# zju-pi/diff-sampler

Measured on NVIDIA H100. Metric: images/sec at fixed NFE, higher is better.
Workload: dtype fp16 operands, fp32 accumulate (split-precision: fp16 hi x hi + two e4m3 correction MMAs per product); 1 GPU; EDM cifar10 U-Net, heun num_steps=10 (NFE=18), batch 512/GPU; net=cifar10, solver=heun, nfe=18, batch_per_gpu=512, global_batch=512, weights=random init (reference constructors, seed 0), init_zero layers de-zeroed, parallelism=dp1, l2=per-forward activation working set (GBs) >> 50 MB L2

## Files before the change

### diff-sampler_b200/_lib.py

```python
import ctypes as C
import os

import torch

from . import _cstructs as S

_HERE = os.path.dirname(os.path.abspath(__file__))
LIB_PATH = os.path.join(_HERE, 'libdiffsampler_b200.so')

EXPORTS = [
    'ds_version', 'ds_last_error', 'ds_weights_create', 'ds_weights_destroy', 'ds_unet_create', 'ds_unet_destroy',
    'ds_unet_forward', 'ds_unet_debug_read', 'ds_unet_last_launch_count', 'ds_solver_update', 'ds_dyn_threshold',
    'ds_op_launch', 'ds_sizeof', 'ds_unet_set_profiling', 'ds_unet_get_profile', 'ds_unet_op_type', 'ds_gits_cost', 'ds_unet_forward_io', 'ds_images_to_uint8', 'ds_solver_update_u8', 'ds_unet_enable_graph', 'ds_amed_predict',
    'ds_gemm_config', 'ds_op_check',
]

_lib = None


class DsError(RuntimeError):
    pass


def load():
    global _lib
    if _lib is not None:
        return _lib
    if not os.path.exists(LIB_PATH):
        raise DsError(f'{LIB_PATH} not found: build it with `python diff-sampler_b200/build.py` '
                      '(there is no CPU fallback for the CUDA path)')
    lib = C.CDLL(LIB_PATH)
    vp, cp, sz = C.c_void_p, C.c_char_p, C.c_size_t
    lib.ds_version.restype = cp
    lib.ds_last_error.restype = cp
    lib.ds_weights_create.argtypes = [vp, sz, C.POINTER(vp)]
    lib.ds_weights_destroy.argtypes = [vp]
    lib.ds_weights_destroy.restype = None
    lib.ds_unet_create.argtypes = [vp, vp, C.c_int, sz, sz, C.POINTER(vp)]
    lib.ds_unet_destroy.argtypes = [vp]
    lib.ds_unet_destroy.restype = None
    lib.ds_unet_forward.argtypes = [vp, vp, vp, vp, vp, vp, vp]
    lib.ds_unet_forward_io.argtypes = [vp, C.POINTER(vp), C.c_int, vp]
    lib.ds_unet_enable_graph.argtypes = [vp, C.POINTER(sz), C.c_int]
    lib.ds_unet_debug_read.argtypes = [vp, sz, vp, sz, vp]
    lib.ds_unet_last_launch_count.argtypes = [vp]
    lib.ds_unet_set_profiling.argtypes = [vp, C.c_int]
    lib.ds_unet_get_profile.argtypes = [vp, C.POINTER(C.c_float), C.c_int]
    lib.ds_unet_op_type.argtypes = [vp, C.c_int]
    lib.ds_solver_update.argtypes = [vp, vp, vp, vp, vp, C.POINTER(vp), C.c_int, vp, C.c_int, C.c_float, vp,
                                     C.POINTER(C.c_float), vp, C.c_int64, C.c_int, vp]
    lib.ds_solver_update_u8.argtypes = [vp, vp, vp, C.c_int, C.c_int, vp, vp, vp, C.POINTER(vp), C.c_int, vp, C.c_int, C.c_float, vp,
                                        C.POINTER(C.c_float), vp, C.c_int64, C.c_int, vp]
    lib.ds_amed_predict.argtypes = [vp, C.POINTER(C.c_int), vp, vp, vp, C.c_float, C.c_float, vp, C.c_int, vp]
    lib.ds_dyn_threshold.argtypes = [vp, vp, C.c_int, C.c_int, C.c_float, C.c_float, vp]
    lib.ds_gits_cost.argtypes = [vp, vp, vp, vp, C.c_int, C.c_int, C.c_int64, vp]
    lib.ds_images_to_uint8.argtypes = [vp, vp, C.c_int, C.c_int, C.c_int, vp]
    lib.ds_op_launch.argtypes = [C.c_int, vp, sz, vp]
    lib.ds_op_check.argtypes = [C.c_int, vp, sz]
    lib.ds_sizeof.argtypes = [C.c_int]
    lib.ds_sizeof.restype = sz
    lib.ds_gemm_config.argtypes = [vp, C.POINTER(C.c_int)]
    for which, cls in S.SIZEOF_CHECKS.items():
        got, want = C.sizeof(cls), lib.ds_sizeof(which)
        if got != want:
            raise DsError(f'struct mirror {cls.__name__}: ctypes size {got} != library size {want}')
    _lib = lib
    return lib


def check(rc, what=''):
    if rc != 0:
        msg = load().ds_last_error().decode()
        raise DsError(f'{what} failed (rc={rc}): {msg}')


def version():
    return load().ds_version().decode()


def op_launch(desc, stream=0):
    lib = load()
    check(lib.ds_op_launch(S.OP_TYPE_OF[type(desc)], C.byref(desc), C.sizeof(desc), C.c_void_p(stream)), type(desc).__name__)


def op_check(desc):
    lib = load()
    if lib.ds_op_check(S.OP_TYPE_OF[type(desc)], C.byref(desc), C.sizeof(desc)) == 0:
        return None
    return lib.ds_last_error().decode()


def gemm_config(desc):
    info = (C.c_int * 2)()
    check(load().ds_gemm_config(C.byref(desc), info), 'ds_gemm_config')
    return dict(stages=info[0], grid=info[1])


class NativePlans:

    def __init__(self, blob, device):
        self.lib = load()
        self.device = device
        self.plans = {}
        self._wh = C.c_void_p()
        with torch.cuda.device(device):
            check(self.lib.ds_weights_create(blob, len(blob), C.byref(self._wh)), 'ds_weights_create')

    def get(self, key, compile_fn, io_bytes=None):
        ent = self.plans.get(key)
        if ent is None:
            pl = compile_fn()
            h = C.c_void_p()
            with torch.cuda.device(self.device):
                check(self.lib.ds_unet_create(self._wh, C.cast(pl.ops_array, C.c_void_p), pl.n_ops, C.sizeof(S.PlanOp), pl.arena_bytes,
                                              C.byref(h)), 'ds_unet_create')
                if io_bytes is not None:
                    check(self.lib.ds_unet_enable_graph(h, (C.c_size_t * S.DS_IO_COUNT)(*io_bytes(pl)), S.DS_IO_COUNT),
                          'ds_unet_enable_graph')
            ent = self.plans[key] = (h, pl)
        return ent

    def run(self, h, io, stream):
        check(self.lib.ds_unet_forward_io(h, (C.c_void_p * S.DS_IO_COUNT)(*io), S.DS_IO_COUNT, C.c_void_p(stream)), 'ds_unet_forward_io')
        return self.lib.ds_unet_last_launch_count(h)

    def debug_read(self, key, name, numel, dtype=torch.float32):
        h, pl = self.plans[key]
        t = torch.empty(numel, dtype=dtype)
        stream = torch.cuda.current_stream(self.device).cuda_stream
        check(self.lib.ds_unet_debug_read(h, pl.arena_offsets[name], t.data_ptr(), t.numel() * t.element_size(), C.c_void_p(stream)),
              'ds_unet_debug_read')
        return t

    def __del__(self):
        try:
            for h, _ in self.plans.values():
                self.lib.ds_unet_destroy(h)
            self.lib.ds_weights_destroy(self._wh)
        except Exception:
            pass
```

### diff-sampler_b200/csrc/gemm_tc.cu

```cuda
#include "ops.h"
#include "ptx.cuh"
#include <cuda_fp16.h>
#include <stdio.h>
#include <stdlib.h>
#include <string.h>

namespace dsb {

static constexpr int kMaxStages = 8;
static constexpr int kATileBytes = 128 * 128;
static constexpr int kThreads = 384;
static constexpr int kStgPitch = 64;
static constexpr int kStgBytes = 2 * 64 * kStgPitch * 4;
static constexpr int kSmemLimit = 227 * 1024;

struct alignas(64) GemmKernelParams {
    CUtensorMap tmA, tmA2, tmB;
    CUtensorMap tmA8, tmA2_8, tmB8;
    int f8, cpb8, nkb8_main, nkb8_aux, a8_plane_n;
    float acc_scale;
    int BN, m_tiles, n_tiles, num_z, nh;
    int taps, cpb, nkb_main, nkb_aux, npass;
    int a_mode, conv_H, conv_W, a_bn_dummy;
    int a_plane_n, a2_plane_n, b_plane_batch;
    int a_c_per_zh, a_n_per_zb, a_n_per_zh;
    int b_k0, b_k_per_zh, b_row_per_zh, b_z_per_zb, b_z_per_zh;
    int m_valid, n_valid;
    int num_stages;
    float* out_f32;
    __half* out_h16;
    long long o_zb, o_zh, ldo, o_plane;
    const float* bias_n;
    const float* bias_m;
    const float* rowvec;
    long long rowvec_stride;
    int rows_per_sample;
    const float* residual;
    long long ldr;
    float scale;
    int edm_out;
    const float* edm_x;
    const float* edm_coef;
    int edm_coef_stride;
    int edm_C;
    float* edm_D;
    float* st_quads;
    int st_unit;
    int tap_dh[9], tap_dw[9], tap_cb[9];
    int f8_last_steps;
};

struct SmemCtl {
    uint64_t full[kMaxStages];
    uint64_t empty[kMaxStages];
};

template <int N>
__device__ __forceinline__ void warp_sum_levels(float* v, int lane, int off) {
    if constexpr (N >= 1) {
        const bool up = (lane & off) != 0;
#pragma unroll
        for (int i = 0; i < N; ++i) {
            const float send = up ? v[i] : v[i + N];
            const float keep = up ? v[i + N] : v[i];
            v[i] = keep + __shfl_xor_sync(0xffffffffu, send, off);
        }
        warp_sum_levels<N / 2>(v, lane, off >> 1);
    } else {
        for (; off >= 1; off >>= 1) v[0] += __shfl_xor_sync(0xffffffffu, v[0], off);
    }
}
template <int NV>
__device__ __forceinline__ void warp_sum_multi(float (&v)[NV], int lane) {
    static_assert(NV == 32 || NV == 16 || NV == 8, "NV");
    warp_sum_levels<NV / 2>(v, lane, 16);
}

template <int W>
__device__ __forceinline__ void epilogue_chunk(const GemmKernelParams& p, const float* v, long long grow_in_z, int col0, bool row_ok,
                                               int zb, int zh) {
    const bool warp_rows_ok = __all_sync(0xffffffffu, row_ok);
    if (!row_ok) return;
    float r[W];
#pragma unroll
    for (int j = 0; j < W; ++j) r[j] = v[j] * p.acc_scale;
    const bool full = (col0 + W <= p.n_valid);
    if (p.bias_n) {
        if (full) {
#pragma unroll
            for (int j = 0; j < W; j += 4) {
                const float4 t = __ldg(reinterpret_cast<const float4*>(p.bias_n + col0 + j));
                r[j] += t.x; r[j + 1] += t.y; r[j + 2] += t.z; r[j + 3] += t.w;
            }
        } else {
#pragma unroll
            for (int j = 0; j < W; ++j)
                if (col0 + j < p.n_valid) r[j] += __ldg(p.bias_n + col0 + j);
        }
    }
    if (p.bias_m) {
        const float bm = __ldg(p.bias_m + grow_in_z);
#pragma unroll
        for (int j = 0; j < W; ++j) r[j] += bm;
    }
    if (p.rowvec) {
        const long long s = (p.rowvec_stride == 0) ? 0 : (grow_in_z / p.rows_per_sample) * p.rowvec_stride;
        const float* rv = p.rowvec + s + col0;
        if (full) {
#pragma unroll
            for (int j = 0; j < W; j += 4) {
                const float4 t = __ldg(reinterpret_cast<const float4*>(rv + j));
                r[j] += t.x; r[j + 1] += t.y; r[j + 2] += t.z; r[j + 3] += t.w;
            }
        } else {
#pragma unroll
            for (int j = 0; j < W; ++j)
                if (col0 + j < p.n_valid) r[j] += __ldg(rv + j);
        }
    }
    if (p.residual) {
        const float* rs = p.residual + grow_in_z * p.ldr + col0;
        if (full) {
#pragma unroll
            for (int j = 0; j < W; j += 4) {
                const float4 t = *reinterpret_cast<const float4*>(rs + j);
                r[j] += t.x; r[j + 1] += t.y; r[j + 2] += t.z; r[j + 3] += t.w;
            }
        } else {
#pragma unroll
            for (int j = 0; j < W; ++j)
                if (col0 + j < p.n_valid) r[j] += rs[j];
        }
    }
#pragma unroll
    for (int j = 0; j < W; ++j) r[j] *= p.scale;

    if (p.st_quads) {
        const int lane = threadIdx.x & 31;
        if (p.st_unit == 2) {
            float q[W];
#pragma unroll
            for (int j = 0; j < W; j += 2) {
                q[j] = r[j] + r[j + 1];
                q[j + 1] = fmaf(r[j], r[j], r[j + 1] * r[j + 1]);
            }
            warp_sum_multi<W>(q, lane);
            constexpr int kShift = (W == 32) ? 0 : 1;
            const int vi = lane >> kShift;
            if ((lane & ((1 << kShift) - 1)) == 0 && col0 + 2 * (vi >> 1) < p.n_valid)
                p.st_quads[(grow_in_z >> 5) * (long long)p.n_valid + col0 + vi] = q[0];
        } else {
            float q[W / 2];
#pragma unroll
            for (int j = 0; j < W; j += 4) {
                q[j / 2] = (r[j] + r[j + 1]) + (r[j + 2] + r[j + 3]);
                q[j / 2 + 1] = fmaf(r[j], r[j], r[j + 1] * r[j + 1]) + fmaf(r[j + 2], r[j + 2], r[j + 3] * r[j + 3]);
            }
            warp_sum_multi<W / 2>(q, lane);
            constexpr int kShift = (W == 32) ? 1 : 2;
            const int vi = lane >> kShift;
            if ((lane & ((1 << kShift) - 1)) == 0 && col0 + 4 * (vi >> 1) < p.n_valid)
                p.st_quads[((grow_in_z >> 5) * (long long)(p.n_valid >> 2)) * 2 + (col0 >> 1) + vi] = q[0];
        }
    }

    if (p.edm_out) {
        const int HW = p.rows_per_sample;
        const long long n = grow_in_z / HW;
        const long long hw = grow_in_z % HW;
        if (p.edm_out == 2) {
#pragma unroll
            for (int j = 0; j < W; ++j) {
                const int c = col0 + j;
                if (c < p.edm_C) p.edm_D[(n * p.edm_C + c) * HW + hw] = r[j];
            }
            return;
        }
        const float cskip = __ldg(p.edm_coef + n * p.edm_coef_stride + 0);
        const float cout = __ldg(p.edm_coef + n * p.edm_coef_stride + 1);
#pragma unroll
        for (int j = 0; j < W; ++j) {
            const int c = col0 + j;
            if (c < p.edm_C) {
                const long long idx = (n * p.edm_C + c) * HW + hw;
                p.edm_D[idx] = cskip * __ldg(p.edm_x + idx) + cout * r[j];
            }
        }
        return;
    }

    const long long obase = (long long)zb * p.o_zb + (long long)zh * p.o_zh + grow_in_z * p.ldo + col0;
    const int odd = threadIdx.x & 1;
    if (p.out_f32) {
        float* o = p.out_f32 + obase;
        if (full && warp_rows_ok) {
            float* oe = o - odd * p.ldo + odd * 4;
#pragma unroll
            for (int j = 0; j < W; j += 8) {
                float x[4];
#pragma unroll
                for (int k = 0; k < 4; ++k) x[k] = __shfl_xor_sync(0xffffffffu, odd ? r[j + k] : r[j + 4 + k], 1);
                const float4 s1 = odd ? make_float4(x[0], x[1], x[2], x[3]) : make_float4(r[j], r[j + 1], r[j + 2], r[j + 3]);
                const float4 s2 = odd ? make_float4(r[j + 4], r[j + 5], r[j + 6], r[j + 7]) : make_float4(x[0], x[1], x[2], x[3]);
                *reinterpret_cast<float4*>(oe + j) = s1;
                *reinterpret_cast<float4*>(oe + p.ldo + j) = s2;
            }
        } else if (full) {
#pragma unroll
            for (int j = 0; j < W; j += 4) *reinterpret_cast<float4*>(o + j) = make_float4(r[j], r[j + 1], r[j + 2], r[j + 3]);
        } else {
#pragma unroll
            for (int j = 0; j < W; ++j)
                if (col0 + j < p.n_valid) o[j] = r[j];
        }
    }
    if (p.out_h16) {
        __half* oh = p.out_h16 + obase;
        if (full) {
            __align__(16) __half hi[W];
            __align__(16) __half lo[W];
#pragma unroll
            for (int j = 0; j < W; ++j) {
                hi[j] = __float2half_rn(r[j]);
                lo[j] = __float2half_rn(r[j] - __half2float(hi[j]));
            }
            if (warp_rows_ok && W % 16 == 0) {
                __half* he = oh - odd * p.ldo + odd * 8;
#pragma unroll
                for (int pl = 0; pl < 2; ++pl) {
                    if (pl == 1 && !p.o_plane) break;
                    const __half* src = pl ? lo : hi;
                    __half* dst = he + (pl ? p.o_plane : 0);
#pragma unroll
                    for (int j = 0; j < W; j += 16) {
                        const uint4 a = *reinterpret_cast<const uint4*>(src + j), b = *reinterpret_cast<const uint4*>(src + j + 8);
                        const uint4 snd = odd ? a : b;
                        uint4 x;
                        x.x = __shfl_xor_sync(0xffffffffu, snd.x, 1); x.y = __shfl_xor_sync(0xffffffffu, snd.y, 1);
                        x.z = __shfl_xor_sync(0xffffffffu, snd.z, 1); x.w = __shfl_xor_sync(0xffffffffu, snd.w, 1);
                        *reinterpret_cast<uint4*>(dst + j) = odd ? x : a;
                        *reinterpret_cast<uint4*>(dst + p.ldo + j) = odd ? b : x;
                    }
                }
            } else {
#pragma unroll
                for (int j = 0; j < W; j += 8) *reinterpret_cast<uint4*>(oh + j) = *reinterpret_cast<const uint4*>(hi + j);
                if (p.o_plane) {
#pragma unroll
                    for (int j = 0; j < W; j += 8)
                        *reinterpret_cast<uint4*>(oh + p.o_plane + j) = *reinterpret_cast<const uint4*>(lo + j);
                }
            }
        } else {
#pragma unroll
            for (int j = 0; j < W; ++j)
                if (col0 + j < p.n_valid) {
                    const __half h = __float2half_rn(r[j]);
                    oh[j] = h;
                    if (p.o_plane) oh[p.o_plane + j] = __float2half_rn(r[j] - __half2float(h));
                }
        }
    }
}

struct RingPos {
    int stage;
    uint32_t phase;
};

struct TileCoord {
    int mt, nt, zb, zh;
};

__device__ __forceinline__ TileCoord tile_coord(const GemmKernelParams& p, int tile) {
    const int tiles_per_z = p.m_tiles * p.n_tiles;
    const int z = tile / tiles_per_z;
    const int t2 = tile - z * tiles_per_z;
    TileCoord c;
    c.mt = t2 / p.n_tiles;
    c.nt = t2 - c.mt * p.n_tiles;
    c.zb = z / p.nh;
    c.zh = z - c.zb * p.nh;
    return c;
}

__device__ __forceinline__ void producer_tile(const GemmKernelParams& p, uint8_t* smem, SmemCtl* ctl, RingPos& r, const int block_bytes,
                                              const int aw0, const int ah0, const int an0, const int a_c_off, const int b_k_off,
                                              const int b_row, const int b_z) {
    const uint32_t tx_bytes = (uint32_t)block_bytes;
    auto load = [&](const CUtensorMap* ma, int ac, int aw, int ah, int an, const CUtensorMap* mb, int bk, int bz) {
        mbar_wait_warp(&ctl->empty[r.stage], r.phase ^ 1);
        uint8_t* sa = smem + r.stage * block_bytes;
        uint64_t* full = &ctl->full[r.stage];
        if (elect_one()) {
            mbar_arrive_expect_tx(full, tx_bytes);
            tma_load_4d(ma, full, sa, ac, aw, ah, an);
            tma_load_3d(mb, full, sa + kATileBytes, bk, b_row, bz);
        }
        __syncwarp();
        if (++r.stage == p.num_stages) { r.stage = 0; r.phase ^= 1; }
    };
    if (p.f8) {
        for (int pass8 = 0; pass8 < 2; ++pass8) {
            const int an8 = an0 + pass8 * p.a8_plane_n;
            int bk = 0;
            for (int tap = 0; tap < p.taps; ++tap) {
                const int aw = aw0 + p.tap_dw[tap], ah = ah0 + p.tap_dh[tap];
                for (int cb = 0; cb < p.cpb8; ++cb, bk += 128) load(&p.tmA8, cb * 128, aw, ah, an8, &p.tmB8, bk, pass8);
            }
            for (int j = 0; j < p.nkb8_aux; ++j, bk += 128) load(&p.tmA2_8, j * 128, aw0, ah0, an8, &p.tmB8, bk, pass8);
        }
    }
    const int npass16 = p.f8 ? 1 : p.npass;
    for (int pi = 0; pi < npass16; ++pi) {
        const int pass = npass16 == 3 ? (pi + 1) % 3 : pi;
        const int an = an0 + (pass == 1 ? p.a_plane_n : 0);
        const int an2 = an0 + (pass == 1 ? p.a2_plane_n : 0);
        const int bz = b_z + (pass == 2 ? p.b_plane_batch : 0);
        int bk = b_k_off;
        for (int tap = 0; tap < p.taps; ++tap) {
            const int aw = aw0 + p.tap_dw[tap], ah = ah0 + p.tap_dh[tap];
            const int ac0 = p.tap_cb[tap] + a_c_off;
            for (int cb = 0; cb < p.cpb; ++cb, bk += 64) load(&p.tmA, ac0 + cb * 64, aw, ah, an, &p.tmB, bk, bz);
        }
        for (int j = 0; j < p.nkb_aux; ++j, bk += 64) load(&p.tmA2, j * 64, aw0, ah0, an2, &p.tmB, bk, bz);
    }
}

template <int BN>
__device__ __forceinline__ void mma_tile(const GemmKernelParams& p, uint8_t* smem, SmemCtl* ctl, RingPos& r, const int block_bytes,
                                         const int wg, float (&acc)[BN / 2]) {
    const bool leader = (threadIdx.x & 127) == 0;
    int prev = -1;
    uint32_t scale0 = 0u;
    auto stage = [&](auto f8, auto steps) {
        constexpr bool F8 = decltype(f8)::value;
        constexpr int NS = decltype(steps)::value;
        mbar_wait(&ctl->full[r.stage], r.phase);
        const uint32_t s0 = smem_u32(smem + r.stage * block_bytes);
        const uint64_t da = wgmma_desc_sw128(s0 + wg * 64 * 128);
        const uint64_t db = wgmma_desc_sw128(s0 + kATileBytes);
        wgmma_fence();
#pragma unroll
        for (int k = 0; k < NS; ++k)
            wgmma_ss<BN, F8>(acc, da + 2 * k, db + 2 * k, k > 0 ? 1u : scale0);
        wgmma_commit();
        wgmma_fence_regs(acc);
        wgmma_wait<1>();
        if (prev >= 0 && leader) mbar_arrive(&ctl->empty[prev]);
        prev = r.stage;
        if (++r.stage == p.num_stages) { r.stage = 0; r.phase ^= 1; }
        scale0 = 1u;
    };
    using f8_t = std::true_type;
    using f16_t = std::false_type;
    using full_t = std::integral_constant<int, 4>;
    using half_t = std::integral_constant<int, 2>;
    if (p.f8) {
        const int full8 = p.f8_last_steps == 2 ? p.cpb8 - 1 : p.cpb8;
        for (int pass8 = 0; pass8 < 2; ++pass8) {
            for (int tap = 0; tap < p.taps; ++tap) {
                for (int cb = 0; cb < full8; ++cb) stage(f8_t{}, full_t{});
                if (full8 < p.cpb8) stage(f8_t{}, half_t{});
            }
            for (int j = 0; j < p.nkb8_aux; ++j) stage(f8_t{}, full_t{});
        }
    }
    const int n16 = (p.f8 ? 1 : p.npass) * (p.nkb_main + p.nkb_aux);
    for (int i = 0; i < n16; ++i) stage(f16_t{}, full_t{});
    wgmma_wait<0>();
    wgmma_fence_regs(acc);
    if (prev >= 0 && leader) mbar_arrive(&ctl->empty[prev]);
}

__device__ __forceinline__ uint32_t stg_swz(uint32_t r) { return (((r & 3) << 1) | ((r >> 2) & 1)) << 4; }

__device__ __forceinline__ uint32_t lane_id_here() {
    uint32_t l;
    asm volatile("mov.u32 %0, %%laneid;" : "=r"(l));
    return l;
}
__device__ __forceinline__ void sts_f2(uint32_t a, float x, float y) {
    asm volatile("st.shared.v2.f32 [%0], {%1, %2};" ::"r"(a), "f"(x), "f"(y) : "memory");
}
__device__ __forceinline__ float4 lds_f4(uint32_t a) {
    float4 v;
    asm volatile("ld.shared.v4.f32 {%0, %1, %2, %3}, [%4];" : "=f"(v.x), "=f"(v.y), "=f"(v.z), "=f"(v.w) : "r"(a) : "memory");
    return v;
}

template <int BN>
__device__ __forceinline__ void epilogue_tile(const GemmKernelParams& p, float* stg, const int wg, const TileCoord& tc, const float (&acc)[BN / 2]) {
    const int lane = threadIdx.x & 31;
    const int w = (threadIdx.x >> 5) & 3;
    const int row = 32 * (w & 1) + lane;
    const long long grow = (long long)tc.mt * 128 + wg * 64 + row;
    const bool row_ok = grow < p.m_valid;
    const int ch = 32 * (w >> 1);
#pragma unroll
    for (int c0 = 0; c0 < BN; c0 += 64) {
        uint32_t ln = lane_id_here();
        const uint32_t wkey = smem_u32(stg) + (16 * w + (ln >> 2)) * 256 + ((8 * (ln & 3)) ^ stg_swz(ln >> 2));
#pragma unroll
        for (int g = 0; g < 32; g += 2) {
            const int gi = c0 / 2 + g;
            if (gi < BN / 2) sts_f2((wkey + 2048 * ((g >> 1) & 1)) ^ (32 * (g >> 2)), acc[gi], acc[gi + 1]);
        }
        warpgroup_sync(1 + wg);
        const int width = min(32, BN - c0 - ch);
        const int col0 = tc.nt * BN + c0 + ch;
        ln = lane_id_here();
        const uint32_t rkey = smem_u32(stg) + (32 * (w & 1) + ln) * 256 + 4 * ch + stg_swz(ln);
        if (width >= 32) {
            float v[32];
#pragma unroll
            for (int j = 0; j < 32; j += 4) *reinterpret_cast<float4*>(v + j) = lds_f4(rkey ^ (4 * j));
            if (col0 < p.n_valid) epilogue_chunk<32>(p, v, grow, col0, row_ok, tc.zb, tc.zh);
        } else if (width >= 16) {
            float v[16];
#pragma unroll
            for (int j = 0; j < 16; j += 4) *reinterpret_cast<float4*>(v + j) = lds_f4(rkey ^ (4 * j));
            if (col0 < p.n_valid) epilogue_chunk<16>(p, v, grow, col0, row_ok, tc.zb, tc.zh);
        }
        warpgroup_sync(1 + wg);
    }
}

template <int BN>
__global__ void __launch_bounds__(kThreads, 1) gemm_tc_kernel(const __grid_constant__ GemmKernelParams p) {
    extern __shared__ __align__(1024) uint8_t smem_raw[];
    uint8_t* smem = reinterpret_cast<uint8_t*>((reinterpret_cast<uintptr_t>(smem_raw) + 1023) & ~uintptr_t(1023));
    const int block_bytes = kATileBytes + BN * 128;
    float* stg = reinterpret_cast<float*>(smem + p.num_stages * block_bytes);
    SmemCtl* ctl = reinterpret_cast<SmemCtl*>(smem + p.num_stages * block_bytes + kStgBytes);

    const int warp = threadIdx.x >> 5;
    const int wg = threadIdx.x >> 7;
    const int total_tiles = p.num_z * p.m_tiles * p.n_tiles;

    if (threadIdx.x == 0) {
        tma_prefetch_desc(&p.tmA);
        tma_prefetch_desc(&p.tmB);
        if (p.nkb_aux) tma_prefetch_desc(&p.tmA2);
        if (p.f8) {
            tma_prefetch_desc(&p.tmA8);
            tma_prefetch_desc(&p.tmB8);
            if (p.nkb8_aux) tma_prefetch_desc(&p.tmA2_8);
        }
        for (int s = 0; s < p.num_stages; ++s) {
            mbar_init(&ctl->full[s], 1);
            mbar_init(&ctl->empty[s], 2);
        }
        fence_barrier_init();
    }
    __syncthreads();

    if (wg == 0) {
        asm volatile("setmaxnreg.dec.sync.aligned.u32 40;");
        if (warp == 0) {
            RingPos ring{0, 0u};
            for (int tile = blockIdx.x; tile < total_tiles; tile += gridDim.x) {
                const TileCoord tc = tile_coord(p, tile);
                int aw0, ah0, an0;
                if (p.a_mode == 0) {
                    const int HW = p.conv_H * p.conv_W;
                    const int p0 = tc.mt * 128;
                    an0 = p0 / HW;
                    const int rem = p0 - an0 * HW;
                    ah0 = rem / p.conv_W;
                    aw0 = rem - ah0 * p.conv_W;
                } else {
                    aw0 = tc.mt * 128;
                    ah0 = 0;
                    an0 = tc.zb * p.a_n_per_zb + tc.zh * p.a_n_per_zh;
                }
                const int a_c_off = tc.zh * p.a_c_per_zh;
                const int b_k_off = p.b_k0 + tc.zh * p.b_k_per_zh;
                const int b_row = tc.nt * BN + tc.zh * p.b_row_per_zh;
                const int b_z = tc.zb * p.b_z_per_zb + tc.zh * p.b_z_per_zh;
                producer_tile(p, smem, ctl, ring, block_bytes, aw0, ah0, an0, a_c_off, b_k_off, b_row, b_z);
            }
        }
    } else {
        asm volatile("setmaxnreg.inc.sync.aligned.u32 232;");
        const int cw = wg - 1;
        float* my_stg = stg + cw * 64 * kStgPitch;
        RingPos ring{0, 0u};
        for (int tile = blockIdx.x; tile < total_tiles; tile += gridDim.x) {
            const TileCoord tc = tile_coord(p, tile);
            float acc[BN / 2];
            mma_tile<BN>(p, smem, ctl, ring, block_bytes, cw, acc);
            epilogue_tile<BN>(p, my_stg, cw, tc, acc);
        }
    }
}

typedef CUresult (*EncodeTiledFn)(CUtensorMap*, CUtensorMapDataType, cuuint32_t, void*, const cuuint64_t*, const cuuint64_t*,
                                  const cuuint32_t*, const cuuint32_t*, CUtensorMapInterleave, CUtensorMapSwizzle,
                                  CUtensorMapL2promotion, CUtensorMapFloatOOBfill);

static EncodeTiledFn get_encode_fn() {
    static EncodeTiledFn fn = nullptr;
    if (!fn) {
        void* p = nullptr;
        cudaDriverEntryPointQueryResult q;
        if (cudaGetDriverEntryPoint("cuTensorMapEncodeTiled", &p, cudaEnableDefault, &q) != cudaSuccess || q != cudaDriverEntryPointSuccess)
            return nullptr;
        fn = reinterpret_cast<EncodeTiledFn>(p);
    }
    return fn;
}

static int encode_map_typed(CUtensorMap* m, const void* ptr, int rank, const int64_t* dims, const int64_t* strides_bytes,
                            const int32_t* box, bool bytes8) {
    EncodeTiledFn fn = get_encode_fn();
    if (!fn) return -1;
    cuuint64_t gd[5];
    cuuint64_t gs[4];
    cuuint32_t bx[5];
    cuuint32_t es[5];
    for (int i = 0; i < rank; ++i) { gd[i] = (cuuint64_t)dims[i]; bx[i] = (cuuint32_t)box[i]; es[i] = 1; }
    for (int i = 0; i + 1 < rank; ++i) gs[i] = (cuuint64_t)strides_bytes[i];
    CUresult r = fn(m, bytes8 ? CU_TENSOR_MAP_DATA_TYPE_UINT8 : CU_TENSOR_MAP_DATA_TYPE_FLOAT16, (cuuint32_t)rank, const_cast<void*>(ptr), gd, gs, bx, es, CU_TENSOR_MAP_INTERLEAVE_NONE,
                    CU_TENSOR_MAP_SWIZZLE_128B, CU_TENSOR_MAP_L2_PROMOTION_L2_256B, CU_TENSOR_MAP_FLOAT_OOB_FILL_NONE);
    if (r != CUDA_SUCCESS) {
        fprintf(stderr, "[dsb] cuTensorMapEncodeTiled failed: %d (rank %d dims %lld %lld %lld %lld box %d %d %d %d)\n", (int)r, rank,
                (long long)dims[0], (long long)dims[1], (long long)dims[2], rank > 3 ? (long long)dims[3] : 0LL, box[0], box[1], box[2],
                rank > 3 ? box[3] : 0);
        return -2;
    }
    return 0;
}

int encode_map(CUtensorMap* m, const void* ptr, int rank, const int64_t* dims, const int64_t* strides_bytes, const int32_t* box) {
    return encode_map_typed(m, ptr, rank, dims, strides_bytes, box, false);
}

OpCheck gemm_check(const ds_gemm_desc& d) {
    if (d.BN < 16 || d.BN > 256 || (d.BN % 16) != 0) return {-10, "gemm: BN"};
    if (d.a_box[0] != 64 || d.a_box[1] * d.a_box[2] * d.a_box[3] != 128) return {-11, "gemm: a_box"};
    if (d.npass != 1 && d.npass != 3) return {-12, "gemm: npass"};
    for (int i = 0; i < 4; ++i) if (d.a_dims[i] > (int64_t(1) << 32)) return {-1, "gemm: A tensor map"};
    for (int i = 0; i < 3; ++i) if (d.a_strides[i] % 16 || d.a_strides[i] >= (int64_t(1) << 40)) return {-1, "gemm: A tensor map"};
    if (d.st_unit != 0 && d.st_unit != 2 && d.st_unit != 4) return {-14, "gemm: st_unit"};
    if (d.f8 & 1) {
        if (d.a_mode != 0 || d.num_z != 1 || d.npass != 3 || d.a_plane_n <= 0) return {-16, "gemm: f8"};
        for (int t = 0; t < 9; ++t) if (d.tap_cb[t]) return {-16, "gemm: f8 with tap_cb"};
        if (d.a_dims[0] % 64 || d.a2_c % 64) return {-16, "gemm: f8 channel remainder"};
    }
    if (d.taps != 1 && d.taps != 9) return {-15, "gemm: taps"};
    if (d.a_mode == 0 && d.conv_W > 128 && (d.conv_W % 128 != 0 || d.a_box[1] != 128)) return {-13, "gemm: row segment"};
    if (d.st_quads && (d.num_z != 1 || d.m_valid % 32 != 0 || d.n_valid % (d.st_unit == 2 ? 2 : 4) != 0 || d.edm_out != 0))
        return {-14, "gemm: st_quads"};
    return {0, nullptr};
}

int gemm_build(const ds_gemm_desc* d, GemmKernelParams* kp) {
    memset(kp, 0, sizeof(*kp));
    if (const int rc = gemm_check(*d).rc) return rc;
    if (encode_map(&kp->tmA, d->a_ptr, 4, d->a_dims, d->a_strides, d->a_box)) return -1;
    if (d->a2_c > 0) {
        int64_t dims2[4] = {d->a2_c, d->a_dims[1], d->a_dims[2], d->a_dims[3]};
        int64_t st2[3] = {d->a2_c * 2, d->a2_c * 2 * d->a_dims[1], d->a2_c * 2 * d->a_dims[1] * d->a_dims[2]};
        if (encode_map(&kp->tmA2, d->a2_ptr, 4, dims2, st2, d->a_box)) return -2;
    }
    int32_t bbox[3] = {64, d->BN, 1};
    if (encode_map(&kp->tmB, d->b_ptr, 3, d->b_dims, d->b_strides, bbox)) return -3;

    kp->BN = d->BN; kp->m_tiles = d->m_tiles; kp->n_tiles = d->n_tiles; kp->num_z = d->num_z; kp->nh = d->nh > 0 ? d->nh : 1;
    kp->taps = d->taps; kp->cpb = d->cpb; kp->nkb_main = d->taps * d->cpb; kp->nkb_aux = d->a2_c > 0 ? (int)((d->a2_c + 63) / 64) : 0;
    kp->npass = d->npass; kp->a_mode = d->a_mode; kp->conv_H = d->conv_H; kp->conv_W = d->conv_W;
    kp->a_plane_n = d->a_plane_n; kp->a2_plane_n = d->a2_plane_n; kp->b_plane_batch = d->b_plane_batch;
    kp->a_c_per_zh = d->a_c_per_zh; kp->a_n_per_zb = d->a_n_per_zb; kp->a_n_per_zh = d->a_n_per_zh;
    kp->b_k0 = d->b_k0; kp->b_k_per_zh = d->b_k_per_zh; kp->b_row_per_zh = d->b_row_per_zh;
    kp->b_z_per_zb = d->b_z_per_zb; kp->b_z_per_zh = d->b_z_per_zh;
    kp->m_valid = d->m_valid; kp->n_valid = d->n_valid;
    kp->out_f32 = d->out_f32; kp->out_h16 = reinterpret_cast<__half*>(d->out_h16);
    kp->o_zb = d->o_zb; kp->o_zh = d->o_zh; kp->ldo = d->ldo; kp->o_plane = d->o_plane;
    kp->bias_n = d->bias_n; kp->bias_m = d->bias_m; kp->rowvec = d->rowvec; kp->rowvec_stride = d->rowvec_stride;
    kp->rows_per_sample = d->rows_per_sample > 0 ? d->rows_per_sample : 1;
    kp->residual = d->residual; kp->ldr = d->ldr; kp->scale = d->scale;
    kp->edm_out = d->edm_out; kp->edm_x = d->edm_x; kp->edm_coef = d->edm_coef; kp->edm_coef_stride = d->edm_coef_stride;
    kp->edm_C = d->edm_C; kp->edm_D = d->edm_D;
    kp->st_quads = d->st_quads;
    kp->st_unit = d->st_unit == 2 ? 2 : 4;
    kp->acc_scale = d->acc_scale == 0.f ? 1.f : d->acc_scale;
    if (d->f8 & 1) {
        const int64_t C = d->a_dims[0], Wd = d->a_dims[1], Hd = d->a_dims[2], Bn = d->a_plane_n;
        const int32_t box8[4] = {128, d->a_box[1], d->a_box[2], d->a_box[3]};
        const int64_t dims8[4] = {C, Wd, Hd, 2 * Bn};
        const int64_t st8[3] = {C, Wd * C, Hd * Wd * C};
        const char* a8 = static_cast<const char*>(d->a_ptr) + Bn * Hd * Wd * C * 2;
        if (encode_map_typed(&kp->tmA8, a8, 4, dims8, st8, box8, true)) return -17;
        kp->f8 = 1;
        kp->f8_last_steps = (d->cpb & 1) ? 2 : 4;
        kp->a8_plane_n = (int)Bn;
        kp->cpb8 = (d->cpb + 1) / 2;
        kp->nkb8_main = d->taps * kp->cpb8;
        kp->nkb8_aux = 0;
        if (d->a2_c > 0) {
            const int64_t C2 = d->a2_c;
            const int64_t dims28[4] = {C2, Wd, Hd, 2 * Bn};
            const int64_t st28[3] = {C2, Wd * C2, Hd * Wd * C2};
            const char* a28 = static_cast<const char*>(d->a2_ptr) + Bn * Hd * Wd * C2 * 2;
            if (encode_map_typed(&kp->tmA2_8, a28, 4, dims28, st28, box8, true)) return -18;
            kp->nkb8_aux = (int)((C2 + 127) / 128);
        }
        const int64_t ktot8 = (int64_t)(kp->nkb8_main + kp->nkb8_aux) * 128;
        const int64_t rows = d->b_dims[1];
        const int64_t bd8[3] = {ktot8, rows, 2};
        const int64_t bs8[2] = {ktot8, rows * ktot8};
        const int32_t bbox8[3] = {128, d->BN, 1};
        const char* b8 = static_cast<const char*>(d->b_ptr) + rows * d->b_dims[0] * 2;
        if (encode_map_typed(&kp->tmB8, b8, 3, bd8, bs8, bbox8, true)) return -19;
    }
    for (int t = 0; t < 9; ++t) { kp->tap_dh[t] = d->tap_dh[t]; kp->tap_dw[t] = d->tap_dw[t]; kp->tap_cb[t] = d->tap_cb[t]; }
    const int stage_bytes = kATileBytes + d->BN * 128;
    int ns = (kSmemLimit - 1024 - kStgBytes - (int)sizeof(SmemCtl)) / stage_bytes;
    if (ns > kMaxStages) ns = kMaxStages;
    kp->num_stages = ns;
    return 0;
}

size_t gemm_params_size() { return sizeof(GemmKernelParams); }
void gemm_patch_edm(GemmKernelParams* kp, const float* x, float* D) { kp->edm_x = x; kp->edm_D = D; }

static int g_num_sms[64] = {};
static bool g_attr_set[64][17] = {};

template <int BN>
static int gemm_launch(const GemmKernelParams* kp, cudaStream_t stream, int slot) {
    if (!g_attr_set[slot][BN / 16]) {
        if (cudaFuncSetAttribute(gemm_tc_kernel<BN>, cudaFuncAttributeMaxDynamicSharedMemorySize, kSmemLimit) != cudaSuccess) return -20;
        g_attr_set[slot][BN / 16] = true;
    }
    const size_t smem = (size_t)kp->num_stages * (kATileBytes + BN * 128) + kStgBytes + sizeof(SmemCtl) + 1024;
    const int tiles = kp->num_z * kp->m_tiles * kp->n_tiles;
    const int grid = tiles < g_num_sms[slot] ? tiles : g_num_sms[slot];
    if (grid <= 0) return 0;
    gemm_tc_kernel<BN><<<grid, kThreads, smem, stream>>>(*kp);
    return cudaGetLastError() == cudaSuccess ? 0 : -21;
}

int gemm_run(const GemmKernelParams* kp, cudaStream_t stream) {
    int dev = 0;
    cudaGetDevice(&dev);
    const int slot = (dev < 0 || dev >= 64) ? 0 : dev;
    if (!g_num_sms[slot]) cudaDeviceGetAttribute(&g_num_sms[slot], cudaDevAttrMultiProcessorCount, slot);
    switch (kp->BN / 16) {
        case 1: return gemm_launch<16>(kp, stream, slot);
        case 2: return gemm_launch<32>(kp, stream, slot);
        case 3: return gemm_launch<48>(kp, stream, slot);
        case 4: return gemm_launch<64>(kp, stream, slot);
        case 5: return gemm_launch<80>(kp, stream, slot);
        case 6: return gemm_launch<96>(kp, stream, slot);
        case 7: return gemm_launch<112>(kp, stream, slot);
        case 8: return gemm_launch<128>(kp, stream, slot);
        case 9: return gemm_launch<144>(kp, stream, slot);
        case 10: return gemm_launch<160>(kp, stream, slot);
        case 11: return gemm_launch<176>(kp, stream, slot);
        case 12: return gemm_launch<192>(kp, stream, slot);
        case 13: return gemm_launch<208>(kp, stream, slot);
        case 14: return gemm_launch<224>(kp, stream, slot);
        case 15: return gemm_launch<240>(kp, stream, slot);
        case 16: return gemm_launch<256>(kp, stream, slot);
        default: return -10;
    }
}

}

extern "C" int ds_gemm_launch(const ds_gemm_desc* d, cudaStream_t stream) {
    dsb::GemmKernelParams kp;
    int rc = dsb::gemm_build(d, &kp);
    if (rc) return rc;
    return dsb::gemm_run(&kp, stream);
}

extern "C" int ds_gemm_config(const void* desc, int* info) {
    dsb::GemmKernelParams kp;
    int rc = dsb::gemm_build(static_cast<const ds_gemm_desc*>(desc), &kp);
    if (rc) return rc;
    int dev = 0, sms = 0;
    cudaGetDevice(&dev);
    if (cudaDeviceGetAttribute(&sms, cudaDevAttrMultiProcessorCount, dev) != cudaSuccess) return -20;
    const int tiles = kp.num_z * kp.m_tiles * kp.n_tiles;
    info[0] = kp.num_stages;
    info[1] = tiles < sms ? tiles : sms;
    return 0;
}
```

Baseline: 294.8 images/s.

## Load halo A tiles once per kw and reuse across kh taps in conv GEMM

After: 298.6 images/s (median of 6 runs). 1.01x the previous value.

```diff
diff --git a/diff-sampler_b200/_lib.py b/diff-sampler_b200/_lib.py
--- a/diff-sampler_b200/_lib.py
+++ b/diff-sampler_b200/_lib.py
@@ -91,9 +91,9 @@
 
 
 def gemm_config(desc):
-    info = (C.c_int * 2)()
+    info = (C.c_int * 3)()
     check(load().ds_gemm_config(C.byref(desc), info), 'ds_gemm_config')
-    return dict(stages=info[0], grid=info[1])
+    return dict(stages=info[0], grid=info[1], a_stages=info[2])
 
 
 class NativePlans:
diff --git a/diff-sampler_b200/csrc/gemm_tc.cu b/diff-sampler_b200/csrc/gemm_tc.cu
--- a/diff-sampler_b200/csrc/gemm_tc.cu
+++ b/diff-sampler_b200/csrc/gemm_tc.cu
@@ -1,6 +1,7 @@
 #include "ops.h"
 #include "ptx.cuh"
 #include <cuda_fp16.h>
+#include <algorithm>
 #include <stdio.h>
 #include <stdlib.h>
 #include <string.h>
@@ -48,11 +49,17 @@
     int st_unit;
     int tap_dh[9], tap_dw[9], tap_cb[9];
     int f8_last_steps;
+    int ring_bytes;
+    int halo, num_a_stages, a_ring_off, a_slot_bytes;
+    int halo_wg1_off;
+    int halo_row_bytes;
 };
 
 struct SmemCtl {
     uint64_t full[kMaxStages];
     uint64_t empty[kMaxStages];
+    uint64_t a_full[kMaxStages];
+    uint64_t a_empty[kMaxStages];
 };
 
 template <int N>
@@ -324,6 +331,54 @@
             for (int cb = 0; cb < p.cpb; ++cb, bk += 64) load(&p.tmA, ac0 + cb * 64, aw, ah, an, &p.tmB, bk, bz);
         }
         for (int j = 0; j < p.nkb_aux; ++j, bk += 64) load(&p.tmA2, j * 64, aw0, ah0, an2, &p.tmB, bk, bz);
+    }
+}
+
+__device__ __forceinline__ void producer_tile_halo(const GemmKernelParams& p, uint8_t* smem, SmemCtl* ctl, RingPos& rb, RingPos& ra,
+                                                   const int b_bytes, const int ah0, const int an0, const int b_k_off, const int b_row,
+                                                   const int b_z) {
+    auto load_a = [&](const CUtensorMap* m, int c, int w, int n) {
+        mbar_wait_warp(&ctl->a_empty[ra.stage], ra.phase ^ 1);
+        uint64_t* full = &ctl->a_full[ra.stage];
+        if (elect_one()) {
+            mbar_arrive_expect_tx(full, (uint32_t)p.a_slot_bytes);
+            tma_load_4d(m, full, smem + p.a_ring_off + ra.stage * p.a_slot_bytes, c, w, ah0 - 1, n);
+        }
+        __syncwarp();
+        if (++ra.stage == p.num_a_stages) { ra.stage = 0; ra.phase ^= 1; }
+    };
+    auto load_b = [&](const CUtensorMap* m, int bk, int bz) {
+        mbar_wait_warp(&ctl->empty[rb.stage], rb.phase ^ 1);
+        uint64_t* full = &ctl->full[rb.stage];
+        if (elect_one()) {
+            mbar_arrive_expect_tx(full, (uint32_t)b_bytes);
+            tma_load_3d(m, full, smem + rb.stage * b_bytes, bk, b_row, bz);
+        }
+        __syncwarp();
+        if (++rb.stage == p.num_stages) { rb.stage = 0; rb.phase ^= 1; }
+    };
+    if (p.f8) {
+        const int tap8 = p.cpb8 * 128;
+        for (int pass8 = 0; pass8 < 2; ++pass8) {
+            const int an8 = an0 + pass8 * p.a8_plane_n;
+            for (int kw = 0; kw < 3; ++kw)
+                for (int cb = 0; cb < p.cpb8; ++cb) {
+                    load_a(&p.tmA8, cb * 128, kw - 1, an8);
+                    for (int kh = 0; kh < 3; ++kh) load_b(&p.tmB8, (kh * 3 + kw) * tap8 + cb * 128, pass8);
+                }
+        }
+    }
+    const int npass16 = p.f8 ? 1 : p.npass;
+    const int tap16 = p.cpb * 64;
+    for (int pi = 0; pi < npass16; ++pi) {
+        const int pass = npass16 == 3 ? (pi + 1) % 3 : pi;
+        const int an = an0 + (pass == 1 ? p.a_plane_n : 0);
+        const int bz = b_z + (pass == 2 ? p.b_plane_batch : 0);
+        for (int kw = 0; kw < 3; ++kw)
+            for (int cb = 0; cb < p.cpb; ++cb) {
+                load_a(&p.tmA, cb * 64, kw - 1, an);
+                for (int kh = 0; kh < 3; ++kh) load_b(&p.tmB, b_k_off + (kh * 3 + kw) * tap16 + cb * 64, bz);
+            }
     }
 }
 
@@ -373,6 +428,66 @@
     if (prev >= 0 && leader) mbar_arrive(&ctl->empty[prev]);
 }
 
+template <int BN>
+__device__ __forceinline__ void mma_tile_halo(const GemmKernelParams& p, uint8_t* smem, SmemCtl* ctl, RingPos& rb, RingPos& ra,
+                                              const int wg, float (&acc)[BN / 2]) {
+    const bool leader = (threadIdx.x & 127) == 0;
+    int prev_b = -1, prev_a = -1;
+    uint32_t scale0 = 0u;
+    const uint32_t a_ring = smem_u32(smem + p.a_ring_off);
+    const uint32_t a_wg = wg ? (uint32_t)p.halo_wg1_off : 0u;
+    auto stage = [&](auto f8, auto steps, const int kh) {
+        constexpr bool F8 = decltype(f8)::value;
+        constexpr int NS = decltype(steps)::value;
+        if (kh == 0) mbar_wait(&ctl->a_full[ra.stage], ra.phase);
+        mbar_wait(&ctl->full[rb.stage], rb.phase);
+        const uint64_t da = wgmma_desc_sw128(a_ring + ra.stage * p.a_slot_bytes + a_wg + kh * p.halo_row_bytes);
+        const uint64_t db = wgmma_desc_sw128(smem_u32(smem + rb.stage * (BN * 128)));
+        wgmma_fence();
+#pragma unroll
+        for (int k = 0; k < NS; ++k)
+            wgmma_ss<BN, F8>(acc, da + 2 * k, db + 2 * k, k > 0 ? 1u : scale0);
+        wgmma_commit();
+        wgmma_fence_regs(acc);
+        wgmma_wait<1>();
+        if (leader) {
+            if (prev_b >= 0) mbar_arrive(&ctl->empty[prev_b]);
+            if (prev_a >= 0) mbar_arrive(&ctl->a_empty[prev_a]);
+        }
+        prev_b = rb.stage;
+        if (++rb.stage == p.num_stages) { rb.stage = 0; rb.phase ^= 1; }
+        prev_a = -1;
+        if (kh == 2) {
+            prev_a = ra.stage;
+            if (++ra.stage == p.num_a_stages) { ra.stage = 0; ra.phase ^= 1; }
+        }
+        scale0 = 1u;
+    };
+    using f8_t = std::true_type;
+    using f16_t = std::false_type;
+    using full_t = std::integral_constant<int, 4>;
+    using half_t = std::integral_constant<int, 2>;
+    if (p.f8) {
+        const int full8 = p.f8_last_steps == 2 ? p.cpb8 - 1 : p.cpb8;
+        for (int pass8 = 0; pass8 < 2; ++pass8)
+            for (int kw = 0; kw < 3; ++kw) {
+                for (int cb = 0; cb < full8; ++cb)
+                    for (int kh = 0; kh < 3; ++kh) stage(f8_t{}, full_t{}, kh);
+                if (full8 < p.cpb8)
+                    for (int kh = 0; kh < 3; ++kh) stage(f8_t{}, half_t{}, kh);
+            }
+    }
+    const int n16 = (p.f8 ? 1 : p.npass) * 3 * p.cpb;
+    for (int i = 0; i < n16; ++i)
+        for (int kh = 0; kh < 3; ++kh) stage(f16_t{}, full_t{}, kh);
+    wgmma_wait<0>();
+    wgmma_fence_regs(acc);
+    if (leader) {
+        if (prev_b >= 0) mbar_arrive(&ctl->empty[prev_b]);
+        if (prev_a >= 0) mbar_arrive(&ctl->a_empty[prev_a]);
+    }
+}
+
 __device__ __forceinline__ uint32_t stg_swz(uint32_t r) { return (((r & 3) << 1) | ((r >> 2) & 1)) << 4; }
 
 __device__ __forceinline__ uint32_t lane_id_here() {
@@ -431,8 +546,8 @@
     extern __shared__ __align__(1024) uint8_t smem_raw[];
     uint8_t* smem = reinterpret_cast<uint8_t*>((reinterpret_cast<uintptr_t>(smem_raw) + 1023) & ~uintptr_t(1023));
     const int block_bytes = kATileBytes + BN * 128;
-    float* stg = reinterpret_cast<float*>(smem + p.num_stages * block_bytes);
-    SmemCtl* ctl = reinterpret_cast<SmemCtl*>(smem + p.num_stages * block_bytes + kStgBytes);
+    float* stg = reinterpret_cast<float*>(smem + p.ring_bytes);
+    SmemCtl* ctl = reinterpret_cast<SmemCtl*>(smem + p.ring_bytes + kStgBytes);
 
     const int warp = threadIdx.x >> 5;
     const int wg = threadIdx.x >> 7;
@@ -451,14 +566,18 @@
             mbar_init(&ctl->full[s], 1);
             mbar_init(&ctl->empty[s], 2);
         }
+        for (int s = 0; s < p.num_a_stages; ++s) {
+            mbar_init(&ctl->a_full[s], 1);
+            mbar_init(&ctl->a_empty[s], 2);
+        }
         fence_barrier_init();
     }
     __syncthreads();
 
     if (wg == 0) {
-        asm volatile("setmaxnreg.dec.sync.aligned.u32 40;");
+        asm volatile("setmaxnreg.dec.sync.aligned.u32 48;");
         if (warp == 0) {
-            RingPos ring{0, 0u};
+            RingPos ring{0, 0u}, ring_a{0, 0u};
             for (int tile = blockIdx.x; tile < total_tiles; tile += gridDim.x) {
                 const TileCoord tc = tile_coord(p, tile);
                 int aw0, ah0, an0;
@@ -478,18 +597,20 @@
                 const int b_k_off = p.b_k0 + tc.zh * p.b_k_per_zh;
                 const int b_row = tc.nt * BN + tc.zh * p.b_row_per_zh;
                 const int b_z = tc.zb * p.b_z_per_zb + tc.zh * p.b_z_per_zh;
-                producer_tile(p, smem, ctl, ring, block_bytes, aw0, ah0, an0, a_c_off, b_k_off, b_row, b_z);
+                if (p.halo) producer_tile_halo(p, smem, ctl, ring, ring_a, BN * 128, ah0, an0, b_k_off, b_row, b_z);
+                else producer_tile(p, smem, ctl, ring, block_bytes, aw0, ah0, an0, a_c_off, b_k_off, b_row, b_z);
             }
         }
     } else {
-        asm volatile("setmaxnreg.inc.sync.aligned.u32 232;");
+        asm volatile("setmaxnreg.inc.sync.aligned.u32 224;");
         const int cw = wg - 1;
         float* my_stg = stg + cw * 64 * kStgPitch;
-        RingPos ring{0, 0u};
+        RingPos ring{0, 0u}, ring_a{0, 0u};
         for (int tile = blockIdx.x; tile < total_tiles; tile += gridDim.x) {
             const TileCoord tc = tile_coord(p, tile);
             float acc[BN / 2];
-            mma_tile<BN>(p, smem, ctl, ring, block_bytes, cw, acc);
+            if (p.halo) mma_tile_halo<BN>(p, smem, ctl, ring, ring_a, cw, acc);
+            else mma_tile<BN>(p, smem, ctl, ring, block_bytes, cw, acc);
             epilogue_tile<BN>(p, my_stg, cw, tc, acc);
         }
     }
@@ -555,10 +676,21 @@
     return {0, nullptr};
 }
 
+static bool halo_eligible(const ds_gemm_desc& d) {
+    if (d.a_mode != 0 || d.taps != 9 || d.a2_c != 0 || d.conv_W > 64 || d.conv_W % 8 != 0 || d.a_box[1] != d.conv_W ||
+        d.a_box[1] * d.a_box[2] < 64)
+        return false;
+    for (int t = 0; t < 9; ++t)
+        if (d.tap_cb[t] != 0 || d.tap_dh[t] != t / 3 - 1 || d.tap_dw[t] != t % 3 - 1) return false;
+    return true;
+}
+
 int gemm_build(const ds_gemm_desc* d, GemmKernelParams* kp) {
     memset(kp, 0, sizeof(*kp));
     if (const int rc = gemm_check(*d).rc) return rc;
-    if (encode_map(&kp->tmA, d->a_ptr, 4, d->a_dims, d->a_strides, d->a_box)) return -1;
+    kp->halo = halo_eligible(*d) ? 1 : 0;
+    const int32_t halo_box[4] = {64, d->a_box[1], d->a_box[2] + 2, d->a_box[3]};
+    if (encode_map(&kp->tmA, d->a_ptr, 4, d->a_dims, d->a_strides, kp->halo ? halo_box : d->a_box)) return -1;
     if (d->a2_c > 0) {
         int64_t dims2[4] = {d->a2_c, d->a_dims[1], d->a_dims[2], d->a_dims[3]};
         int64_t st2[3] = {d->a2_c * 2, d->a2_c * 2 * d->a_dims[1], d->a2_c * 2 * d->a_dims[1] * d->a_dims[2]};
@@ -588,10 +720,11 @@
     if (d->f8 & 1) {
         const int64_t C = d->a_dims[0], Wd = d->a_dims[1], Hd = d->a_dims[2], Bn = d->a_plane_n;
         const int32_t box8[4] = {128, d->a_box[1], d->a_box[2], d->a_box[3]};
+        const int32_t halo_box8[4] = {128, d->a_box[1], d->a_box[2] + 2, d->a_box[3]};
         const int64_t dims8[4] = {C, Wd, Hd, 2 * Bn};
         const int64_t st8[3] = {C, Wd * C, Hd * Wd * C};
         const char* a8 = static_cast<const char*>(d->a_ptr) + Bn * Hd * Wd * C * 2;
-        if (encode_map_typed(&kp->tmA8, a8, 4, dims8, st8, box8, true)) return -17;
+        if (encode_map_typed(&kp->tmA8, a8, 4, dims8, st8, kp->halo ? halo_box8 : box8, true)) return -17;
         kp->f8 = 1;
         kp->f8_last_steps = (d->cpb & 1) ? 2 : 4;
         kp->a8_plane_n = (int)Bn;
@@ -615,10 +748,24 @@
         if (encode_map_typed(&kp->tmB8, b8, 3, bd8, bs8, bbox8, true)) return -19;
     }
     for (int t = 0; t < 9; ++t) { kp->tap_dh[t] = d->tap_dh[t]; kp->tap_dw[t] = d->tap_dw[t]; kp->tap_cb[t] = d->tap_cb[t]; }
+    const int budget = kSmemLimit - 1024 - kStgBytes - (int)sizeof(SmemCtl);
+    if (kp->halo) {
+        const int bw = d->a_box[1], bh = d->a_box[2], ipx = bw * bh;
+        const int b_bytes = d->BN * 128;
+        kp->a_slot_bytes = bw * (bh + 2) * d->a_box[3] * 128;
+        kp->num_stages = std::min(kMaxStages, (budget - 2 * kp->a_slot_bytes) / b_bytes);
+        kp->num_a_stages = std::min(kMaxStages, (budget - kp->num_stages * b_bytes) / kp->a_slot_bytes);
+        kp->a_ring_off = kp->num_stages * b_bytes;
+        kp->ring_bytes = kp->a_ring_off + kp->num_a_stages * kp->a_slot_bytes;
+        kp->halo_row_bytes = bw * 128;
+        kp->halo_wg1_off = ((64 / ipx) * (bh + 2) * bw + 64 % ipx) * 128;
+        return 0;
+    }
     const int stage_bytes = kATileBytes + d->BN * 128;
-    int ns = (kSmemLimit - 1024 - kStgBytes - (int)sizeof(SmemCtl)) / stage_bytes;
+    int ns = budget / stage_bytes;
     if (ns > kMaxStages) ns = kMaxStages;
     kp->num_stages = ns;
+    kp->ring_bytes = ns * stage_bytes;
     return 0;
 }
 
@@ -634,7 +781,7 @@
         if (cudaFuncSetAttribute(gemm_tc_kernel<BN>, cudaFuncAttributeMaxDynamicSharedMemorySize, kSmemLimit) != cudaSuccess) return -20;
         g_attr_set[slot][BN / 16] = true;
     }
-    const size_t smem = (size_t)kp->num_stages * (kATileBytes + BN * 128) + kStgBytes + sizeof(SmemCtl) + 1024;
+    const size_t smem = (size_t)kp->ring_bytes + kStgBytes + sizeof(SmemCtl) + 1024;
     const int tiles = kp->num_z * kp->m_tiles * kp->n_tiles;
     const int grid = tiles < g_num_sms[slot] ? tiles : g_num_sms[slot];
     if (grid <= 0) return 0;
@@ -687,5 +834,6 @@
     const int tiles = kp.num_z * kp.m_tiles * kp.n_tiles;
     info[0] = kp.num_stages;
     info[1] = tiles < sms ? tiles : sms;
+    info[2] = kp.num_a_stages;
     return 0;
 }
```
